# mihaibujanca/dynamicfusion

Measured on AMD Instinct MI355X. Metric: frames/sec integrate+raycast, 640x480->512^3 TSDF, higher is better.
Workload: dtype f32 (fp16 TSDF / u16 weight storage, f64 exp + normalise as in the reference)

## Files before the change

dynamicfusion_amd/csrc/dfusion_internal.h:

```cpp
#pragma once
#include <hip/hip_runtime.h>
#include <stdint.h>
#include <string.h>
#include <memory>
#include <utility>
#include "dfusion.h"
#include "dfusion_device.h"
#include "dfusion_nanoflann.h"

#define DF_BRICK 8
#define DF_WARP_PREFETCH_MARGIN_M 0.05f
#define DF_WARP_PREFETCH_CAP 1024u

#define DF_HIP(expr) do { hipError_t e__ = (expr); if (e__ != hipSuccess) return (int)e__; } while (0)
#define DF_LAUNCH_CHECK() do { hipError_t e__ = hipGetLastError(); if (e__ != hipSuccess) return (int)e__; } while (0)

static inline DfSlab df_slab_or_full(const DfVolume& v, const DfSlab* s)
{
    if (s) return *s;
    DfSlab f; f.z_store0 = 0; f.z_store_n = v.dims[2]; f.z_own0 = 0; f.z_own_n = v.dims[2]; return f;
}
static inline bool df_slab_valid(const DfVolume& v, const DfSlab& s)
{
    return s.z_store_n > 0 && s.z_own_n >= 0 && s.z_store0 >= 0 && s.z_store0 + s.z_store_n <= v.dims[2] &&
// ... 71 lines not shown
    unsigned long long plan_reader[2] = {};
    DfDevBuf<unsigned long long> plan_mask2[2]; DfDevBuf<unsigned int> plan_list2[2]; int pphase = 0; unsigned hphase = 0;
    DfDevBuf<unsigned long long> plan_code2[2];
    DfDevBuf<uint16_t> pyr_mem;
    DfDevBuf<char> solver_ws;
    DfDevBuf<int> graph_nbr; DfDevBuf<float> graph_alpha; DfDevBuf<unsigned int> graph_in_off, graph_in_edge; DfDevBuf<char> graph_ws;
    int graph_kg = 0;
    DfDevBuf<int> pt_ids;
    int pt_image_cols = 0;
    DfDevBuf<DfNfNode> nf_nodes; DfDevBuf<uint16_t> nf_vpos; bool nf_ok = false; int nf_depth = 0;
    DfDevBuf<unsigned int> plan_hist; size_t plan_cap = 0;
    DfDevBuf<uint8_t> blk_state; DfDevBuf<float> blk_wmax; DfDevBuf<uint8_t> blk_alive; DfDevBuf<uint32_t> blk_work, blk_cnt; size_t blk_cap = 0; int blk_phase = 0;
    DfDevBuf<uint8_t> blk_tie;
    DfDevBuf<uint16_t> bm_idx; DfDevBuf<uint32_t> bm_lam, bm_w; DfDevBuf<uint8_t> bm_cnt; size_t bm_cap = 0;
    DfDevBuf<uint32_t> code_tab; size_t code_cap = 0; DfDevBuf<uint32_t> bm_ids; DfDevBuf<uint8_t> bm_coded;
    DfDevBuf<uint32_t> bm_sub_lam, bm_sub_w; DfDevBuf<uint16_t> bm_sub_cnt; DfDevBuf<uint8_t> bm_sub_ok, blk_sub, blk_alive_prev; DfDevBuf<uint32_t> sub_list;
    bool tab_complete = false;
    int tab_sweeps = 0;
    unsigned long long* dbg_swept = nullptr;
    bool alive_valid = false;
    hipStream_t side = nullptr; hipEvent_t ev_fork = nullptr, ev_join = nullptr; bool side_pending = false;
    volatile uint32_t* host_report = nullptr;
    DfDevBuf<char> ext_ws;
    DfDevBuf<char> grow_ws;
};

#define DF_DISPATCH_K(k, ...)                             \
    switch (k) {                                          \
        case 1: { constexpr int K = 1; __VA_ARGS__; } break; \
        case 2: { constexpr int K = 2; __VA_ARGS__; } break; \
        case 3: { constexpr int K = 3; __VA_ARGS__; } break; \
// ... 69 lines not shown
```

dynamicfusion_amd/csrc/dfusion_warp.hip:

```cpp
#include "dfusion_internal.h"
#include "dfusion_pyramid.h"
#include "dfusion_warp_sweep.h"
#include "dfusion_warp_blocks.h"
#include "dfusion_warp_pipe.h"
#include <algorithm>
#include <atomic>
#include <stdlib.h>
#include <stdio.h>
#include <math.h>

__global__ __launch_bounds__(256) void df_dists_max_kernel(const uint16_t* __restrict__ dists, size_t pitch, int cols, int rows,
                                                           float* __restrict__ out)
{
    float m = 0.f;
    for (int i = blockIdx.x * 256 + threadIdx.x; i < cols * rows; i += gridDim.x * 256) {
        const int y = i / cols, x = i - y * cols;
        const float d = h2f_bits(*(const uint16_t*)((const char*)dists + (size_t)y * pitch + 2 * (size_t)x));
        if (!(d <= 3.0e38f)) m = 3.0e38f;
        else m = fmaxf(m, d);
    }
#pragma unroll
    for (int o = 32; o >= 1; o >>= 1) m = fmaxf(m, __shfl_xor(m, o, 64));
    if ((threadIdx.x & 63) == 0) atomicMax((unsigned int*)out, __float_as_uint(m));
}
// ... 132 lines not shown
    wf->blk_phase ^= 1;
    int rc = df_build_listed(wf, cnt, st);
    if (rc) return rc;
    wf->tab_complete = true;
    return DF_OK;
}

static int df_block_verdicts(DfWarpField* wf, DfWarpedArgs& a, int k, unsigned flags, hipStream_t st)
{
    const int nbx = a.tab_ntx * (DF_TAB_TX / 8), nby = a.tab_nty * (DF_TAB_TY / 8), nbz = wf->tab_zn / 8;
    const size_t nblk = (size_t)nbx * nby * nbz;
    if (nblk == 0 || nblk > wf->blk_cap) return DF_E_INVALID;
    const bool use_models = !(flags & DF_WARP_NO_BLOCK_MODEL) && (k == 8 || k == 4);
    const int want_models = !use_models ? 0 : (flags & DF_WARP_BLOCK_MODEL_NOW) ? 2 : wf->tab_sweeps >= 1 ? 1 : 0;
    if (want_models && nblk > wf->bm_cap) {
        wf->bm_cap = 0;
        { int rc = wf->bm_idx.reserve(nblk * DF_BM_NU); if (rc) return rc; }
        { int rc = wf->bm_lam.reserve(nblk * DF_BM_NU); if (rc) return rc; }
        { int rc = wf->bm_w.reserve(nblk * DF_BM_NU); if (rc) return rc; }
        { int rc = wf->bm_cnt.reserve(nblk); if (rc) return rc; }
        wf->bm_cap = nblk;
    }
    if (want_models && k == 8 && (nblk * 512 > wf->code_cap || !wf->bm_ids || !wf->code_tab || !wf->bm_coded || !wf->bm_sub_lam || !wf->bm_sub_w ||
                                  !wf->bm_sub_cnt || !wf->bm_sub_ok || !wf->blk_sub || !wf->sub_list)) {
        wf->code_cap = 0;
        { int rc = wf->bm_ids.reserve(nblk * 64); if (rc) return rc; }
        { int rc = wf->code_tab.reserve(nblk * 512); if (rc) return rc; }
        { int rc = wf->bm_coded.reserve(nblk); if (rc) return rc; }
        DF_HIP(hipMemsetAsync(wf->bm_coded, 0, nblk, st));
        { int rc = wf->bm_sub_lam.reserve(nblk * 8 * DF_BM_NU); if (rc) return rc; }
        { int rc = wf->bm_sub_w.reserve(nblk * 8 * DF_BM_NU); if (rc) return rc; }
        { int rc = wf->bm_sub_cnt.reserve(nblk * 8); if (rc) return rc; }
        { int rc = wf->bm_sub_ok.reserve(nblk); if (rc) return rc; }
        { int rc = wf->blk_sub.reserve(nblk); if (rc) return rc; }
        { int rc = wf->sub_list.reserve(nblk); if (rc) return rc; }
        DF_HIP(hipMemsetAsync(wf->bm_sub_ok, 0, nblk, st));
        wf->code_cap = nblk * 512;
    }
    bool ahead = !(flags & (DF_WARP_NO_PREFETCH | DF_WARP_BLOCK_MODEL_NOW));
    if (ahead) { int rc = df_side_init(wf); if (rc) return rc; }
    if (ahead && !(flags & DF_WARP_STEADY_PREFETCH) && wf->tab_sweeps >= 8 && (wf->tab_sweeps & 7) != 0 && wf->host_report &&
        wf->host_report[0] == 0u && wf->host_report[1] == 0u && wf->host_report[2] == 0u) ahead = false;
    const bool quiet = !ahead && !(flags & (DF_WARP_NO_PREFETCH | DF_WARP_BLOCK_MODEL_NOW));
    const int want_models_policy = want_models;
    const int want_models_now = quiet ? 0 : want_models_policy;
    a.pf_margin = ahead && !wf->tab_complete && wf->tab_sweeps >= 1 ? DF_WARP_PREFETCH_MARGIN_M : 0.f;
    a.pf_cap = DF_WARP_PREFETCH_CAP;
    uint32_t* cnt = wf->blk_cnt + 8 * wf->blk_phase;
    uint32_t* cnt_next = wf->blk_cnt + 8 * (wf->blk_phase ^ 1);
    uint32_t* list_urgent = wf->blk_work, *list_ahead = wf->blk_work + wf->blk_cap, *list_model = wf->blk_work + 2 * wf->blk_cap;
    std::swap(wf->blk_alive, wf->blk_alive_prev);
    const bool codes_exist = k == 8 && wf->bm_cnt && wf->code_tab && wf->bm_ids && wf->bm_coded && wf->code_cap >= nblk * 512;
    const bool sub_verdicts = use_models && wf->bm_cap >= nblk && codes_exist && !(flags & DF_WARP_NO_SUB_VERDICT) && wf->bm_sub_lam && wf->bm_sub_w &&
                              wf->bm_sub_cnt && wf->bm_sub_ok && wf->blk_sub && wf->sub_list && wf->blk_alive_prev;
    if (sub_verdicts) { a.bm_ids = wf->bm_ids; a.bm_sub_lam = wf->bm_sub_lam; a.bm_sub_w = wf->bm_sub_w; a.bm_sub_cnt = wf->bm_sub_cnt; a.bm_sub_ok = wf->bm_sub_ok; }
    hipLaunchKernelGGL(df_block_verdict_kernel, dim3((unsigned)((nblk + 255) / 256)), dim3(256), 0, st, a, wf->rot, wf->node_t, nbx, nby, nbz,
                       wf->blk_state, wf->blk_wmax, wf->brick_thr + wf->off_cap, wf->bx, wf->by, a.tile_wmax != nullptr ? 1 : 0,
                       (use_models && wf->bm_cap >= nblk ? 1 : 0) | (codes_exist ? 2 : 0) | (sub_verdicts ? 4 : 0),
                       want_models_now,
                       wf->tab_complete ? 0 : 1, wf->bm_idx, wf->bm_lam, wf->bm_w, wf->bm_cnt, wf->bm_coded, wf->blk_alive, list_urgent, list_ahead, list_model,
                       cnt, cnt_next, sub_verdicts ? (uint8_t*)wf->blk_sub : nullptr, wf->sub_list, wf->blk_alive_prev);
    a.blk_cnt = cnt; a.host_report = (uint32_t*)wf->host_report; a.sweep_no = (uint32_t)wf->tab_sweeps;
    DF_LAUNCH_CHECK();
#ifdef DF_TRACE_VERDICT
    if (getenv("DF_TRACE_VERDICT_FILE")) {
        DF_HIP(hipStreamSynchronize(st));
        static unsigned long long h[8192 * 4];
        DF_HIP(hipMemcpyFromSymbol(h, HIP_SYMBOL(g_df_vtrace), sizeof(h)));
        FILE* f = fopen(getenv("DF_TRACE_VERDICT_FILE"), "wb");
        if (f) { fwrite(h, 8, 8192 * 4, f); fclose(f); }
    }
#endif
    wf->blk_phase ^= 1;
    auto launch_models = [&](hipStream_t s2) -> int {
        const DfWarpedArgs b = df_table_args(wf);
        static unsigned g8 = 0, g4 = 0;
// ... 6 lines not shown
                                wf->bm_idx, wf->bm_lam, wf->bm_w, wf->bm_cnt, wf->blk_state);
        DF_LAUNCH_CHECK();
        return DF_OK;
    };
    const bool side_work = ahead && (!wf->tab_complete || want_models_now);
    if (side_work) {
        DF_HIP(hipEventRecord(wf->ev_fork, st));
        DF_HIP(hipStreamWaitEvent(wf->side, wf->ev_fork, 0));
        int rc_side = DF_OK;
        if (!wf->tab_complete) rc_side = df_build_listed(wf, cnt, wf->side, 1);
        if (rc_side == DF_OK && want_models_now) rc_side = launch_models(wf->side);
        if (hipEventRecord(wf->ev_join, wf->side) == hipSuccess) wf->side_pending = true;
        else { (void)hipGetLastError(); df_side_drain(wf); if (rc_side == DF_OK) rc_side = (int)hipErrorUnknown; }
        if (rc_side != DF_OK) return rc_side;
    }
    if (sub_verdicts) {
        const unsigned sub_grid = (unsigned)std::min<size_t>((nblk * 8 + 255) / 256, 1024);
        hipLaunchKernelGGL(df_sub_verdict_kernel, dim3(sub_grid), dim3(256), 0, st, a, wf->rot, wf->node_t, nbx, nby, nbz, wf->sub_list, cnt + 5, wf->blk_sub);
        DF_LAUNCH_CHECK();
        a.blk_sub = wf->blk_sub;
    }
    if (!wf->tab_complete) { int rc = df_build_listed(wf, cnt, st, 0); if (rc) return rc; }
    if (want_models_now && !ahead) { int rc = launch_models(st); if (rc) return rc; }
    a.blk_alive = wf->blk_alive; a.bm_nbx = nbx; a.bm_nby = nby;
    wf->alive_valid = true;
    return DF_OK;
}

typedef void (*df_lds_kernel_t)(const DfWarpedArgs, const DfWarpView, int);
struct DfPrepared { DfWarpedArgs a; DfWarpView W; df_lds_kernel_t kern; dim3 grid; unsigned threads; size_t lds; int tiles_x; DfVolume v; DfSlab s; unsigned long long seq; };
DfWarpField::DfWarpField() = default;
DfWarpField::~DfWarpField() = default;
enum { DF_MODE_WHOLE = 0, DF_MODE_PREPARE = 1 };

static int df_integrate_warped_impl(const uint16_t* dists, size_t pitch, int cols, int rows, DfVolume v, const DfSlab* slab,
                                    const float vol2world[12], const float world2cam[12], const float proj[4],
// ... 53 lines not shown
                                    const float vol2world[12], const float world2cam[12], const float proj[4],
                                    DfWarpField* wf, int k, unsigned flags, unsigned long long* n_updated, dfStream stream, int mode)
{
    if (!dists || !vol2world || !world2cam || !proj || !wf || cols <= 0 || rows <= 0 || !df_pitch_ok(pitch, cols, 2) || !df_volume_valid(v)) return DF_E_INVALID;
    if (k < 1 || k > 8 || wf->M < k) return DF_E_INVALID;
    DfSlab s = df_slab_or_full(v, slab);
    if (!df_slab_valid(v, s)) return DF_E_INVALID;
    if (!wf->index_valid || wf->k_built < k || memcmp(wf->geom_dims, v.dims, sizeof(wf->geom_dims)) ||
        memcmp(wf->geom_vs, v.voxel_size, sizeof(wf->geom_vs)) || memcmp(wf->geom_aff, vol2world, sizeof(wf->geom_aff)))
        return DF_E_NO_INDEX;
    if (s.z_own_n == 0) return DF_OK;
    hipStream_t st = (hipStream_t)stream;
    if (mode == DF_MODE_WHOLE) { int rc = df_wait_split_sweep(wf, st); if (rc) return rc; }
    { int rc = df_side_join(wf, st); if (rc) return rc; }
    wf->prep_valid = false;

    DfWarpedArgs a;
    memset(&a, 0, sizeof(a));
    a.vol = (uint32_t*)v.data; a.X = v.dims[0]; a.Y = v.dims[1]; a.Z = v.dims[2];
    a.z_store0 = s.z_store0; a.z_own0 = s.z_own0; a.z_own_n = s.z_own_n;
    a.vsx = v.voxel_size[0]; a.vsy = v.voxel_size[1]; a.vsz = v.voxel_size[2];
    a.vol2world = df_aff(vol2world); a.world2cam = df_aff(world2cam);
    {
        static const float I9[9] = {1.f, 0.f, 0.f, 0.f, 1.f, 0.f, 0.f, 0.f, 1.f};
        a.v2w_identity = memcmp(vol2world, I9, sizeof(I9)) == 0;
    }
    a.P.dists = dists; a.P.pitch = pitch; a.P.cols = cols; a.P.rows = rows;
    a.P.fx = proj[0]; a.P.fy = proj[1]; a.P.cx = proj[2]; a.P.cy = proj[3];
    a.P.trunc = v.trunc_dist; a.P.trunc_inv = 1.f / v.trunc_dist; a.P.max_weight = v.max_weight;
    a.sat_ok = df_sat_trunc_ok(v.trunc_dist) ? 1 : 0;
// ... 199 lines not shown
    if (weights) {
        { int rc = wf->tile_wmax.reserve(ntile); if (rc) return rc; }
        DF_HIP(hipMemsetAsync(wf->tile_wmax, 0, ntile * sizeof(float), st));
    }
    const size_t nblk = (size_t)ntx * (DF_TAB_TX / 8) * nty * (DF_TAB_TY / 8) * (tzn / 8);
    if (nblk > wf->blk_cap) {
        wf->blk_cap = 0;
        { int rc = wf->blk_state.reserve(nblk); if (rc) return rc; }
        { int rc = wf->blk_tie.reserve(nblk); if (rc) return rc; }
        { int rc = wf->blk_wmax.reserve(nblk); if (rc) return rc; }
        { int rc = wf->blk_alive.reserve(nblk); if (rc) return rc; }
        { int rc = wf->blk_alive_prev.reserve(nblk); if (rc) return rc; }
        { int rc = wf->blk_work.reserve(3 * nblk); if (rc) return rc; }
        wf->blk_cap = nblk;
    }
    { int rc = wf->blk_cnt.reserve(16); if (rc) return rc; }
    DF_HIP(hipMemsetAsync(wf->blk_cnt, 0, 16 * sizeof(uint32_t), st));
    DF_HIP(hipMemsetAsync(wf->blk_state, on_demand ? 0 : 1, nblk, st));
    DF_HIP(hipMemsetAsync(wf->blk_tie, 0, nblk, st));
    DF_HIP(hipMemsetAsync(wf->blk_wmax, 0, nblk * sizeof(float), st));
    DF_HIP(hipMemsetAsync(wf->blk_alive, 1, nblk, st));
    DF_HIP(hipMemsetAsync(wf->blk_alive_prev, 1, nblk, st));
    wf->blk_phase = 0;
    wf->tab_z0 = tz0; wf->tab_zn = tzn; wf->tab_k = k; wf->tab_valid = true; wf->w_tab_valid = weights;
    wf->tab_complete = !on_demand; wf->tab_sweeps = 0; wf->alive_valid = false;
    if (on_demand) return DF_OK;
    const DfWarpedArgs a = df_table_args(wf);
    DfWarpView W = df_view(wf);
    dim3 grid((unsigned)(W.bx * W.by), (unsigned)(bz_hi - bz_lo + 1));
    DF_DISPATCH_K(k, df_warp_brick_kernel<K, true><<<grid, dim3(256), 0, st>>>(a, W));
    hipError_t e = hipGetLastError();
    if (e == hipSuccess) e = hipStreamSynchronize(st);
// ... 7 lines not shown
```

dynamicfusion_amd/csrc/dfusion_warp_blocks.h:

```cpp
#pragma once
#include "dfusion_warp_sweep.h"

#define DF_BM_NU 16
#define DF_BM_NONE 0xffu

struct DfIv { float lo, hi; };
__device__ __forceinline__ DfIv iv(float lo, float hi) { DfIv r; r.lo = lo; r.hi = hi; return r; }
__device__ __forceinline__ DfIv iv_add(DfIv a, DfIv b) { return iv(a.lo + b.lo, a.hi + b.hi); }
__device__ __forceinline__ DfIv iv_sub(DfIv a, DfIv b) { return iv(a.lo - b.hi, a.hi - b.lo); }
__device__ __forceinline__ DfIv iv_mul(DfIv a, DfIv b)
{
    const float p0 = a.lo * b.lo, p1 = a.lo * b.hi, p2 = a.hi * b.lo, p3 = a.hi * b.hi;
    return iv(fminf(fminf(p0, p1), fminf(p2, p3)), fmaxf(fmaxf(p0, p1), fmaxf(p2, p3)));
}
__device__ __forceinline__ DfIv iv_sq(DfIv a)
{
    const float l2 = a.lo * a.lo, h2 = a.hi * a.hi;
    return iv((a.lo <= 0.f && a.hi >= 0.f) ? 0.f : fminf(l2, h2), fmaxf(l2, h2));
}
struct DfIv3 { DfIv x, y, z; };
__device__ __forceinline__ DfIv3 iv_cross(const DfIv3& a, const DfIv3& b)
{
    DfIv3 r;
    r.x = iv_sub(iv_mul(a.y, b.z), iv_mul(a.z, b.y));
// ... 285 lines not shown
        for (int i = 0; i < 4; ++i) {
            const size_t at = (size_t)min(e0 + (unsigned)i, n - 1u) * nblk + blk;
            id[i] = bm_idx[at]; lp[i] = bm_lam[at]; wp[i] = bm_w[at];
        }
        float4 r4[4], t4[4];
#pragma unroll
        for (int i = 0; i < 4; ++i) { r4[i] = rot[id[i]]; t4[i] = node_t[id[i]]; }
#pragma unroll
        for (int i = 0; i < 4; ++i) B.add(e0 + (unsigned)i < n, lp[i], wp[i], r4[i], t4[i]);
    }
    const int bx = (int)(blk % (size_t)nbx), by = (int)((blk / (size_t)nbx) % (size_t)nby), bz = (int)(blk / ((size_t)nbx * nby));
    const int x0 = bx * 8, y0 = by * 8, z0 = a.tab_z0 + bz * 8;
    return df_box_dead_finish(a, B, x0, min(x0 + 7, a.X - 1), y0, min(y0 + 7, a.Y - 1), z0, min(z0 + 7, a.Z - 1));
}

__global__ __launch_bounds__(256) void df_sub_verdict_kernel(const DfWarpedArgs a, const float4* __restrict__ rot, const float4* __restrict__ node_t,
                                                             int nbx, int nby, int nbz, const uint32_t* __restrict__ list, const uint32_t* __restrict__ count,
                                                             uint8_t* __restrict__ blk_sub)
{
    const size_t nblk = (size_t)nbx * nby * nbz;
    const unsigned n_lanes = min(*count, (uint32_t)nblk) * 8u;
    for (unsigned base = blockIdx.x * 256u + (threadIdx.x & ~63u); base < n_lanes; base += gridDim.x * 256u) {
    const unsigned i = base + (threadIdx.x & 63u);
    const bool in = i < n_lanes;
    size_t blk = in ? (size_t)list[i >> 3] : 0;
    if (blk >= nblk) blk = 0;
    const unsigned sub = i & 7u, h = sub >> 2, q = sub & 3u;
    const unsigned cr = a.bm_sub_cnt[blk * 8 + sub];
    const uint4* idp = (const uint4*)(a.bm_ids + blk * 64 + q * 16);
    const uint4 i0 = idp[0], i1 = idp[1], i2 = idp[2], i3 = idp[3];
    const unsigned idw[DF_BM_NU] = {i0.x, i0.y, i0.z, i0.w, i1.x, i1.y, i1.z, i1.w, i2.x, i2.y, i2.z, i2.w, i3.x, i3.y, i3.z, i3.w};
    uint32_t lp[DF_BM_NU], wp[DF_BM_NU];
    const size_t at0 = blk * (8 * DF_BM_NU) + sub;
#pragma unroll
    for (int e = 0; e < DF_BM_NU; ++e) { lp[e] = a.bm_sub_lam[at0 + 8 * e]; wp[e] = a.bm_sub_w[at0 + 8 * e]; }
    const unsigned n = in ? min(cr & 0xffu, (unsigned)DF_BM_NU) : 0u, e_ref = min(cr >> 8, (unsigned)DF_BM_NU - 1u);
    unsigned id[DF_BM_NU], id_ref = 0u;
#pragma unroll
    for (int e = 0; e < DF_BM_NU; ++e) {
        id[e] = (unsigned)e < n ? (idw[e] >> (16u * h)) & 0xffffu : 0u;
        id_ref = (unsigned)e == e_ref ? id[e] : id_ref;
    }
    bool live = n != 0u;
    const bool judge = in && n != 0u && a.cull[1] <= 1.0f;
    DfBoxSums B;
    B.ref(rot[id_ref]);
#pragma unroll
    for (int g = 0; g < DF_BM_NU; g += 8) {
        if (g != 0 && __builtin_amdgcn_ballot_w64(judge && n > (unsigned)g) == 0ull) break;
        float4 r4[8], t4[8];
#pragma unroll
        for (int j = 0; j < 8; ++j) { r4[j] = rot[id[g + j]]; t4[j] = node_t[id[g + j]]; }
#pragma unroll
        for (int j = 0; j < 8; ++j) if ((unsigned)(g + j) < n) B.add(true, lp[g + j], wp[g + j], r4[j], t4[j]);
    }
    if (judge) {
        const int bx = (int)(blk % (size_t)nbx), by = (int)((blk / (size_t)nbx) % (size_t)nby), bz = (int)(blk / ((size_t)nbx * nby));
        const int x0 = bx * 8 + (int)(q & 1u) * 4, y0 = by * 8 + (int)(q >> 1) * 4, z0 = a.tab_z0 + bz * 8 + (int)h * 4;
        if (x0 < a.X && y0 < a.Y && z0 < a.Z)
            live = !df_box_dead_finish(a, B, x0, min(x0 + 3, a.X - 1), y0, min(y0 + 3, a.Y - 1), z0, min(z0 + 3, a.Z - 1));
        else live = false;
    }
    const unsigned long long m = __builtin_amdgcn_ballot_w64(live);
    if (in && sub == 0u) blk_sub[blk] = (uint8_t)((unsigned)(m >> ((threadIdx.x & 63u) & ~7u)) & 0xffu);
    }
}

#ifdef DF_TRACE_VERDICT
__device__ unsigned long long g_df_vtrace[8192 * 4];
#define DF_VT(i) do { if ((threadIdx.x & 63) == 0 && blockIdx.x * 4 + (threadIdx.x >> 6) < 8192) g_df_vtrace[(blockIdx.x * 4 + (threadIdx.x >> 6)) * 4 + (i)] = wall_clock64(); } while (0)
#else
#define DF_VT(i) do { } while (0)
#endif
__global__ __launch_bounds__(256) void df_block_verdict_kernel(const DfWarpedArgs a, const float4* __restrict__ rot, const float4* __restrict__ node_t,
                                                               int nbx, int nby, int nbz, uint8_t* __restrict__ blk_state,
                                                               const float* __restrict__ blk_wmax, const float* __restrict__ brick_d1, int vbx, int vby, int zero_skip, int use_models, int want_models,
                                                               int build_on_demand, const uint16_t* __restrict__ bm_idx,
                                                               const uint32_t* __restrict__ bm_lam, const uint32_t* __restrict__ bm_w,
                                                               const uint8_t* __restrict__ bm_cnt, const uint8_t* __restrict__ bm_coded, uint8_t* __restrict__ alive,
                                                               uint32_t* __restrict__ build_list, uint32_t* __restrict__ ahead_list, uint32_t* __restrict__ model_list,
                                                               uint32_t* __restrict__ cnt, uint32_t* __restrict__ cnt_next,
                                                               uint8_t* __restrict__ blk_sub, uint32_t* __restrict__ sub_list, const uint8_t* __restrict__ alive_prev)
{
    __shared__ unsigned s_sub_n, s_sub_base;
    if (threadIdx.x == 0) s_sub_n = 0u;
    const size_t nblk = (size_t)nbx * nby * nbz;
    const size_t blk = (size_t)blockIdx.x * 256 + threadIdx.x;
    DF_VT(0);
    if (blockIdx.x == 0 && threadIdx.x < 8) cnt_next[threadIdx.x] = 0u;
    bool keep = false, near = false, need_build = false, need_ahead = false, need_model = false, need_sub = false;
    int bx = 0, by = 0, bz = 0;
    if (blk < nblk) {
        bx = (int)(blk % (size_t)nbx); by = (int)((blk / (size_t)nbx) % (size_t)nby); bz = (int)(blk / ((size_t)nbx * nby));
        const int x0 = bx * 8, y0 = by * 8, z0 = a.tab_z0 + bz * 8;
        const int own1 = min(a.z_own0 + a.z_own_n, a.Z);
        keep = x0 < a.X && y0 < a.Y && max(z0, a.z_own0) < min(z0 + 8, own1);
        const unsigned st = keep ? blk_state[blk] : 0u;
        if (keep) {
            float wk = a.kf;
            if (zero_skip && st >= 1u) {
                const float wmax = blk_wmax[blk];
                keep = !(wmax * a.cull[3] < DF_ZERO_WEIGHT);
                wk = fminf(wk, wmax * 1.0001f);
            } else if (zero_skip && a.cull[4] < 1.0e30f && a.cull[4] > 0.f) {
// ... 6 lines not shown
            if (keep) {
                const f3 c = aff_mul(a.vol2world, mk3(((float)x0 + 3.5f) * a.vsx, ((float)y0 + 3.5f) * a.vsy, ((float)z0 + 3.5f) * a.vsz));
                if (a.pf_margin > 0.f && st < 2u) {
                    near = !df_tile_culled(a, c, wk, a.pf_margin);
                    keep = near && !df_tile_culled(a, c, wk);
                } else keep = !df_tile_culled(a, c, wk);
            }
        }
        DF_VT(1);
        if (keep && st == 2u && (use_models & 1)) {
            const unsigned n = bm_cnt[blk];
            if (n != DF_BM_NONE && a.cull[1] <= 1.0f) keep = !df_block_box_dead(a, rot, node_t, nbx, nby, nblk, blk, n, bm_idx, bm_lam, bm_w);
        }
        DF_VT(2);
        alive[blk] = keep ? (uint8_t)(1u | ((st == 2u && (use_models & 2) && bm_coded[blk] != 0) ? 2u : 0u)) : (uint8_t)0;
        if (blk_sub) {
            blk_sub[blk] = 0xffu;
            if (keep && st == 2u && (use_models & 4) && a.bm_sub_ok[blk] != 0) {
                const size_t sy = (size_t)nbx, sz = (size_t)nbx * nby;
                const unsigned n0 = bx > 0 ? alive_prev[blk - 1] : 1u, n1 = bx + 1 < nbx ? alive_prev[blk + 1] : 1u, n2 = by > 0 ? alive_prev[blk - sy] : 1u,
                               n3 = by + 1 < nby ? alive_prev[blk + sy] : 1u, n4 = bz > 0 ? alive_prev[blk - sz] : 1u, n5 = bz + 1 < nbz ? alive_prev[blk + sz] : 1u;
                need_sub = n0 == 0u || n1 == 0u || n2 == 0u || n3 == 0u || n4 == 0u || n5 == 0u;
            }
        }
        need_build = keep && build_on_demand && st == 0u;
        need_ahead = !keep && near && build_on_demand && st == 0u;
        need_model = (keep || near) && want_models && (st == 1u || (need_build && want_models > 1));
        if (need_build) blk_state[blk] = 1;
    }
    const unsigned long long mb = __builtin_amdgcn_ballot_w64(need_build), ma = __builtin_amdgcn_ballot_w64(need_ahead), mm = __builtin_amdgcn_ballot_w64(need_model);
    const unsigned long long below = ((unsigned long long)1 << (threadIdx.x & 63)) - 1ull;
    const unsigned code = (unsigned)bx | ((unsigned)by << 10) | ((unsigned)(a.tab_z0 / 8 + bz) << 20);
// ... 4 lines not shown
        if (need_build) build_list[base + (unsigned)__popcll(mb & below)] = code;
    }
    if (ma) {
        unsigned base = 0;
        if ((threadIdx.x & 63) == 0) base = atomicAdd(&cnt[3], (unsigned)__popcll(ma));
        base = (unsigned)__builtin_amdgcn_readfirstlane((int)base);
        const unsigned slot = base + (unsigned)__popcll(ma & below);
        if (need_ahead && slot < a.pf_cap) { ahead_list[slot] = code; blk_state[blk] = 1; }
    }
    if (mm) {
        unsigned base = 0;
        if ((threadIdx.x & 63) == 0) base = atomicAdd(&cnt[1], (unsigned)__popcll(mm));
        base = (unsigned)__builtin_amdgcn_readfirstlane((int)base);
        if (need_model) model_list[base + (unsigned)__popcll(mm & below)] = (unsigned)blk;
    }
    if (blk_sub) {
        const unsigned long long ms = __builtin_amdgcn_ballot_w64(need_sub);
        unsigned wbase = 0;
        __syncthreads();
        if (ms && (threadIdx.x & 63) == 0) wbase = atomicAdd(&s_sub_n, (unsigned)__popcll(ms));
        wbase = (unsigned)__builtin_amdgcn_readfirstlane((int)wbase);
        __syncthreads();
        if (threadIdx.x == 0 && s_sub_n) s_sub_base = atomicAdd(&cnt[5], s_sub_n);
        __syncthreads();
        if (need_sub) sub_list[s_sub_base + wbase + (unsigned)__popcll(ms & below)] = (unsigned)blk;
    }
    DF_VT(3);
}

__global__ __launch_bounds__(256) void df_blocks_unbuilt_kernel(int nbx, int nby, int nbz, int vbx, int vby, int tab_bz0, uint8_t* __restrict__ blk_state,
                                                                uint32_t* __restrict__ build_list, uint32_t* __restrict__ cnt,
                                                                uint32_t* __restrict__ cnt_next)
{
    const size_t nblk = (size_t)nbx * nby * nbz;
    const size_t blk = (size_t)blockIdx.x * 256 + threadIdx.x;
    if (blockIdx.x == 0 && threadIdx.x < 8) cnt_next[threadIdx.x] = 0u;
    bool need = false;
    int bx = 0, by = 0, bz = 0;
    if (blk < nblk) {
        bx = (int)(blk % (size_t)nbx); by = (int)((blk / (size_t)nbx) % (size_t)nby); bz = (int)(blk / ((size_t)nbx * nby));
        need = blk_state[blk] == 0 && bx < vbx && by < vby;
        if (blk_state[blk] == 0) blk_state[blk] = 1;
// ... 11 lines not shown
```

dynamicfusion_amd/csrc/dfusion_warp_index.hip:

```cpp
#include "dfusion_internal.h"
#include "dfusion_warp_sweep.h"
#include <math.h>

struct DfIndexGeom {
    int X, Y, Z; int bx, by, bz;
    float vsx, vsy, vsz;
    DfAff vol2world;
    float r2x;
};

#define DF_SUPER 4
#define DF_SUPER_CAP 1024
template <int K>
__device__ __forceinline__ float df_wave_kth_pop(float (&bd)[K], float* first)
{
    const int lane = threadIdx.x & 63;
    float dk2 = 0.f;
#pragma unroll
    for (int r = 0; r < K; ++r) {
        const float m = wave_min_f32(bd[0]);
        dk2 = m;
        if (r == 0) *first = m;
        const unsigned long long who = __ballot(bd[0] == m);
        const int first = __ffsll((long long)who) - 1;
// ... 238 lines not shown
        for (int i = 0; i < 3; ++i)
            wf->geom_inv[9 + i] = (float)-((d[3 * i] * m[9] + d[3 * i + 1] * m[10] + d[3 * i + 2] * m[11]) / det);
    }
    return DF_OK;
}

extern "C" int dfusion_warp_build_index(DfWarpField* wf, DfVolume v, const DfSlab* slab, const float vol2world[12], int k,
                                        unsigned flags, dfStream stream)
{
    if (!wf || !vol2world || wf->M <= 0 || k < 1 || k > 8 || wf->M < k) return DF_E_INVALID;
    if (v.dims[0] <= 0 || v.dims[1] <= 0 || v.dims[2] <= 0) return DF_E_INVALID;
    DfSlab sl = df_slab_or_full(v, slab);
    if (sl.z_own_n < 0 || sl.z_own0 < 0 || sl.z_own0 + sl.z_own_n > v.dims[2]) return DF_E_INVALID;
    hipStream_t st = (hipStream_t)stream;
    df_side_drain(wf);
    wf->prep_valid = false;
    { int rc = df_index_bricks(wf, v, vol2world, k, st); if (rc) return rc; }
    wf->index_flags = flags; wf->index_slab = sl;
    wf->index_valid = true;
    wf->tab_valid = false;
    wf->w_tab_valid = false;
    if (flags & (DF_INDEX_VOXEL_TABLE | DF_INDEX_WEIGHT_TABLE))
        return df_build_voxel_table(wf, v, sl, vol2world, k, (flags & DF_INDEX_WEIGHT_TABLE) != 0,
                                    (flags & DF_INDEX_TABLES_ON_DEMAND) != 0 && (flags & DF_INDEX_WEIGHT_TABLE) != 0, st);
    return DF_OK;
}

extern "C" int dfusion_warp_index_info(const DfWarpField* wf, unsigned long long* total_entries, unsigned int* n_bricks, int* k_built)
{
    if (!wf || !wf->index_valid) return DF_E_NO_INDEX;
// ... 55 lines not shown
    }
    wf->index_valid = false;
    DfVolume v; memset(&v, 0, sizeof(v));
    memcpy(v.dims, wf->geom_dims, sizeof(v.dims)); memcpy(v.voxel_size, wf->geom_vs, sizeof(v.voxel_size));
    float aff[12]; memcpy(aff, wf->geom_aff, sizeof(aff));
    { int rc = df_index_bricks(wf, v, aff, wf->k_built, st); if (rc) return rc; }
    wf->index_valid = true;
    if (!tabs) return DF_OK;
    const DfWarpedArgs a = df_table_args(wf);
    const int nbz = wf->tab_zn / 8;
    const size_t nblk = (size_t)a.bm_nbx * a.bm_nby * nbz;
    hipLaunchKernelGGL(df_grow_dirty_kernel, dim3((unsigned)((nblk + 255) / 256)), dim3(256), 0, st, old_off, old_list, wf->brick_off, wf->brick_list,
                       wf->bx, wf->by, wf->bz, a.bm_nbx, a.bm_nby, nbz, wf->tab_z0 / DF_BRICK, wf->blk_state, a.blk_wmax, wf->blk_tie);
    DF_LAUNCH_CHECK();
    wf->alive_valid = false; wf->tab_complete = false;
    if (!((wf->index_flags & DF_INDEX_TABLES_ON_DEMAND) && wf->w_tab_valid)) {
        int rc = df_tables_complete(wf, st);
        if (rc) return rc;
    }
    DF_HIP(hipStreamSynchronize(st));
    return DF_OK;
}
```

dynamicfusion_amd/csrc/dfusion_warp_nodes.hip:

```cpp
#include "dfusion_internal.h"
#include <utility>
#include <vector>

__global__ __launch_bounds__(256) void df_pack_nodes_kernel(const float* __restrict__ pos, const float* __restrict__ dq,
                                                            const float* __restrict__ sigma, int M,
                                                            float4* __restrict__ pos_sigma, float4* __restrict__ rot,
                                                            float4* __restrict__ dual, float4* __restrict__ node_t, float4* __restrict__ rt)
{
    int j = blockIdx.x * 256 + threadIdx.x;
    if (j >= M) return;
    if (pos) pos_sigma[j] = make_float4(pos[3 * j], pos[3 * j + 1], pos[3 * j + 2], sigma[j]);
    quat r, d;
    r.w = dq[8 * j]; r.x = dq[8 * j + 1]; r.y = dq[8 * j + 2]; r.z = dq[8 * j + 3];
    d.w = dq[8 * j + 4]; d.x = dq[8 * j + 5]; d.y = dq[8 * j + 6]; d.z = dq[8 * j + 7];
    quat t = dq_get_translation(r, d);
    rot[j] = make_float4(r.w, r.x, r.y, r.z);
    dual[j] = make_float4(d.w, d.x, d.y, d.z);
    node_t[j] = make_float4(t.w, t.x, t.y, t.z);
    rt[2 * j] = rot[j]; rt[2 * j + 1] = node_t[j];
}

__global__ __launch_bounds__(256) void df_node_bounds_kernel(const float4* __restrict__ rot, const float4* __restrict__ node_t,
                                                             int M, float* __restrict__ bounds)
{
// ... 217 lines not shown
    return DF_OK;
}

extern "C" int dfusion_warp_set_nodes(DfWarpField* wf, const float* pos, const float* dq, const float* sigma, int M,
                                      dfStream stream)
{
    if (!wf || !pos || !dq || !sigma || M <= 0 || M > 65535) return DF_E_INVALID;
    df_side_drain(wf);
    wf->prep_valid = false;
    int rc = df_warp_reserve(wf, M);
    if (rc) return rc;
    wf->M = M;
    wf->graph_kg = 0;
    wf->index_valid = false;
    wf->tab_valid = false; wf->w_tab_valid = false;
    rc = df_warp_pack(wf, pos, dq, sigma, (hipStream_t)stream);
    if (rc) return rc;
    return df_warp_build_tie_tree(wf, (hipStream_t)stream);
}

extern "C" int dfusion_warp_set_transforms(DfWarpField* wf, const float* dq, dfStream stream)
{
    if (!wf || !dq || wf->M <= 0) return DF_E_INVALID;
    return df_warp_pack(wf, nullptr, dq, nullptr, (hipStream_t)stream);
}

DfWarpView df_view(const DfWarpField* wf)
{
    DfWarpView W;
    W.pos_sigma = wf->pos_sigma; W.rot = wf->rot; W.dual = wf->dual; W.node_t = wf->node_t; W.rt = wf->rt; W.M = wf->M;
// ... 5 lines not shown
```

Measured before the change: 2013.

## Fuse sub-verdict into block-verdict launch using previous call's sub list

Removes the separate sub-verdict kernel launch. The block-verdict kernel now gets extra workgroups that judge sub-blocks using the list built in the previous call. That list is kept in double-buffered sub lists and blk_sub arrays, with rotating counters, and an invalidation key forces a fallback whenever geometry, nodes or call order change. The sub-verdict loop is also rewritten to prefetch node ids, lambdas and weights in groups of four, and it adds a blk_state check. The cost is that verdicts lag one call behind the list, so blocks that newly qualify stay conservatively fully live (0xff) for that call, and state management gets more complex.

```diff
diff --git a/dynamicfusion_amd/csrc/dfusion_internal.h b/dynamicfusion_amd/csrc/dfusion_internal.h
--- a/dynamicfusion_amd/csrc/dfusion_internal.h
+++ b/dynamicfusion_amd/csrc/dfusion_internal.h
@@ -109,7 +109,8 @@
     DfDevBuf<uint8_t> blk_tie;
     DfDevBuf<uint16_t> bm_idx; DfDevBuf<uint32_t> bm_lam, bm_w; DfDevBuf<uint8_t> bm_cnt; size_t bm_cap = 0;
     DfDevBuf<uint32_t> code_tab; size_t code_cap = 0; DfDevBuf<uint32_t> bm_ids; DfDevBuf<uint8_t> bm_coded;
-    DfDevBuf<uint32_t> bm_sub_lam, bm_sub_w; DfDevBuf<uint16_t> bm_sub_cnt; DfDevBuf<uint8_t> bm_sub_ok, blk_sub, blk_alive_prev; DfDevBuf<uint32_t> sub_list;
+    DfDevBuf<uint32_t> bm_sub_lam, bm_sub_w; DfDevBuf<uint16_t> bm_sub_cnt; DfDevBuf<uint8_t> bm_sub_ok, blk_sub2[2], blk_alive_prev; DfDevBuf<uint32_t> sub_list2[2];
+    unsigned judge_no = 0; bool sub_void = true; int judge_key[6] = {}; unsigned long long call_no = 0, judge_call = 0;
     bool tab_complete = false;
     int tab_sweeps = 0;
     unsigned long long* dbg_swept = nullptr;
diff --git a/dynamicfusion_amd/csrc/dfusion_warp.hip b/dynamicfusion_amd/csrc/dfusion_warp.hip
--- a/dynamicfusion_amd/csrc/dfusion_warp.hip
+++ b/dynamicfusion_amd/csrc/dfusion_warp.hip
@@ -170,7 +170,7 @@
     const bool use_models = !(flags & DF_WARP_NO_BLOCK_MODEL) && (k == 8 || k == 4);
     const int want_models = !use_models ? 0 : (flags & DF_WARP_BLOCK_MODEL_NOW) ? 2 : wf->tab_sweeps >= 1 ? 1 : 0;
     if (want_models && nblk > wf->bm_cap) {
-        wf->bm_cap = 0;
+        wf->bm_cap = 0; wf->sub_void = true;
         { int rc = wf->bm_idx.reserve(nblk * DF_BM_NU); if (rc) return rc; }
         { int rc = wf->bm_lam.reserve(nblk * DF_BM_NU); if (rc) return rc; }
         { int rc = wf->bm_w.reserve(nblk * DF_BM_NU); if (rc) return rc; }
@@ -178,7 +178,7 @@
         wf->bm_cap = nblk;
     }
     if (want_models && k == 8 && (nblk * 512 > wf->code_cap || !wf->bm_ids || !wf->code_tab || !wf->bm_coded || !wf->bm_sub_lam || !wf->bm_sub_w ||
-                                  !wf->bm_sub_cnt || !wf->bm_sub_ok || !wf->blk_sub || !wf->sub_list)) {
+                                  !wf->bm_sub_cnt || !wf->bm_sub_ok || !wf->blk_sub2[0] || !wf->blk_sub2[1] || !wf->sub_list2[0] || !wf->sub_list2[1])) {
         wf->code_cap = 0;
         { int rc = wf->bm_ids.reserve(nblk * 64); if (rc) return rc; }
         { int rc = wf->code_tab.reserve(nblk * 512); if (rc) return rc; }
@@ -188,8 +188,12 @@
         { int rc = wf->bm_sub_w.reserve(nblk * 8 * DF_BM_NU); if (rc) return rc; }
         { int rc = wf->bm_sub_cnt.reserve(nblk * 8); if (rc) return rc; }
         { int rc = wf->bm_sub_ok.reserve(nblk); if (rc) return rc; }
-        { int rc = wf->blk_sub.reserve(nblk); if (rc) return rc; }
-        { int rc = wf->sub_list.reserve(nblk); if (rc) return rc; }
+        wf->sub_void = true;
+        for (int i = 0; i < 2; ++i) {
+            { int rc = wf->blk_sub2[i].reserve(nblk); if (rc) return rc; }
+            { int rc = wf->sub_list2[i].reserve(nblk); if (rc) return rc; }
+            DF_HIP(hipMemsetAsync(wf->blk_sub2[i], 0xff, wf->blk_sub2[i].cap, st));
+        }
         DF_HIP(hipMemsetAsync(wf->bm_sub_ok, 0, nblk, st));
         wf->code_cap = nblk * 512;
     }
@@ -208,14 +212,36 @@
     std::swap(wf->blk_alive, wf->blk_alive_prev);
     const bool codes_exist = k == 8 && wf->bm_cnt && wf->code_tab && wf->bm_ids && wf->bm_coded && wf->code_cap >= nblk * 512;
     const bool sub_verdicts = use_models && wf->bm_cap >= nblk && codes_exist && !(flags & DF_WARP_NO_SUB_VERDICT) && wf->bm_sub_lam && wf->bm_sub_w &&
-                              wf->bm_sub_cnt && wf->bm_sub_ok && wf->blk_sub && wf->sub_list && wf->blk_alive_prev;
+                              wf->bm_sub_cnt && wf->bm_sub_ok && wf->blk_sub2[0] && wf->blk_sub2[1] && wf->sub_list2[0] && wf->sub_list2[1] && wf->blk_alive_prev &&
+                              wf->blk_cnt.cap >= 19;
     if (sub_verdicts) { a.bm_ids = wf->bm_ids; a.bm_sub_lam = wf->bm_sub_lam; a.bm_sub_w = wf->bm_sub_w; a.bm_sub_cnt = wf->bm_sub_cnt; a.bm_sub_ok = wf->bm_sub_ok; }
-    hipLaunchKernelGGL(df_block_verdict_kernel, dim3((unsigned)((nblk + 255) / 256)), dim3(256), 0, st, a, wf->rot, wf->node_t, nbx, nby, nbz,
-                       wf->blk_state, wf->blk_wmax, wf->brick_thr + wf->off_cap, wf->bx, wf->by, a.tile_wmax != nullptr ? 1 : 0,
-                       (use_models && wf->bm_cap >= nblk ? 1 : 0) | (codes_exist ? 2 : 0) | (sub_verdicts ? 4 : 0),
-                       want_models_now,
-                       wf->tab_complete ? 0 : 1, wf->bm_idx, wf->bm_lam, wf->bm_w, wf->bm_cnt, wf->bm_coded, wf->blk_alive, list_urgent, list_ahead, list_model,
-                       cnt, cnt_next, sub_verdicts ? (uint8_t*)wf->blk_sub : nullptr, wf->sub_list, wf->blk_alive_prev);
+    const unsigned nV = (unsigned)((nblk + 255) / 256);
+    unsigned nS = 0, jn = wf->judge_no;
+    bool list_void = true;
+    if (sub_verdicts) {
+        const int key[6] = {wf->tab_z0, nbx, nby, nbz, a.z_own0, a.z_own_n};
+        list_void = wf->sub_void || wf->judge_call + 1 != wf->call_no || memcmp(key, wf->judge_key, sizeof(key)) != 0;
+        memcpy(wf->judge_key, key, sizeof(key)); wf->judge_call = wf->call_no;
+        if (!list_void) nS = (unsigned)std::min<size_t>((nblk * 8 + 255) / 256, 1024);
+        wf->sub_void = false; ++wf->judge_no;
+    }
+    uint32_t* sub_cnt = wf->blk_cnt + 16;
+    DfJudgeArgs j;
+    memset(&j, 0, sizeof(j));
+    j.rot = wf->rot; j.node_t = wf->node_t; j.nbx = nbx; j.nby = nby; j.nbz = nbz; j.blk_state = wf->blk_state; j.blk_wmax = wf->blk_wmax;
+    j.brick_d1 = wf->brick_thr + wf->off_cap; j.vbx = wf->bx; j.vby = wf->by; j.zero_skip = a.tile_wmax != nullptr ? 1 : 0;
+    j.use_models = (use_models && wf->bm_cap >= nblk ? 1 : 0) | (codes_exist ? 2 : 0) | (sub_verdicts ? 4 : 0);
+    j.want_models = want_models_now; j.build_on_demand = wf->tab_complete ? 0 : 1;
+    j.bm_idx = wf->bm_idx; j.bm_lam = wf->bm_lam; j.bm_w = wf->bm_w; j.bm_cnt = wf->bm_cnt; j.bm_coded = wf->bm_coded; j.alive = wf->blk_alive;
+    j.build_list = list_urgent; j.ahead_list = list_ahead; j.model_list = list_model; j.cnt = cnt; j.cnt_next = cnt_next;
+    j.alive_prev = wf->blk_alive_prev; j.nV = nV; j.list_void = list_void ? 1 : 0;
+    if (sub_verdicts) {
+        j.blk_sub_next = wf->blk_sub2[(jn + 1) & 1]; j.blk_sub_cur = wf->blk_sub2[jn & 1];
+        j.sub_list = wf->sub_list2[jn & 1]; j.sub_cnt_fill = sub_cnt + jn % 3; j.sub_cnt_zero = sub_cnt + (jn + 1) % 3;
+        j.sub_prev = wf->sub_list2[(jn + 1) & 1]; j.sub_cnt_prev = sub_cnt + (jn + 2) % 3;
+    }
+    hipLaunchKernelGGL(df_block_verdict_kernel, dim3(nV + nS), dim3(256), 0, st, a, j);
+    if (sub_verdicts) a.blk_sub = wf->blk_sub2[jn & 1];
     a.blk_cnt = cnt; a.host_report = (uint32_t*)wf->host_report; a.sweep_no = (uint32_t)wf->tab_sweeps;
     DF_LAUNCH_CHECK();
 #ifdef DF_TRACE_VERDICT
@@ -252,12 +278,6 @@
         else { (void)hipGetLastError(); df_side_drain(wf); if (rc_side == DF_OK) rc_side = (int)hipErrorUnknown; }
         if (rc_side != DF_OK) return rc_side;
     }
-    if (sub_verdicts) {
-        const unsigned sub_grid = (unsigned)std::min<size_t>((nblk * 8 + 255) / 256, 1024);
-        hipLaunchKernelGGL(df_sub_verdict_kernel, dim3(sub_grid), dim3(256), 0, st, a, wf->rot, wf->node_t, nbx, nby, nbz, wf->sub_list, cnt + 5, wf->blk_sub);
-        DF_LAUNCH_CHECK();
-        a.blk_sub = wf->blk_sub;
-    }
     if (!wf->tab_complete) { int rc = df_build_listed(wf, cnt, st, 0); if (rc) return rc; }
     if (want_models_now && !ahead) { int rc = launch_models(st); if (rc) return rc; }
     a.blk_alive = wf->blk_alive; a.bm_nbx = nbx; a.bm_nby = nby;
@@ -341,6 +361,7 @@
     if (mode == DF_MODE_WHOLE) { int rc = df_wait_split_sweep(wf, st); if (rc) return rc; }
     { int rc = df_side_join(wf, st); if (rc) return rc; }
     wf->prep_valid = false;
+    ++wf->call_no;
 
     DfWarpedArgs a;
     memset(&a, 0, sizeof(a));
@@ -570,8 +591,9 @@
         { int rc = wf->blk_work.reserve(3 * nblk); if (rc) return rc; }
         wf->blk_cap = nblk;
     }
-    { int rc = wf->blk_cnt.reserve(16); if (rc) return rc; }
-    DF_HIP(hipMemsetAsync(wf->blk_cnt, 0, 16 * sizeof(uint32_t), st));
+    { int rc = wf->blk_cnt.reserve(20); if (rc) return rc; }
+    DF_HIP(hipMemsetAsync(wf->blk_cnt, 0, 20 * sizeof(uint32_t), st));
+    wf->sub_void = true;
     DF_HIP(hipMemsetAsync(wf->blk_state, on_demand ? 0 : 1, nblk, st));
     DF_HIP(hipMemsetAsync(wf->blk_tie, 0, nblk, st));
     DF_HIP(hipMemsetAsync(wf->blk_wmax, 0, nblk * sizeof(float), st));
diff --git a/dynamicfusion_amd/csrc/dfusion_warp_blocks.h b/dynamicfusion_amd/csrc/dfusion_warp_blocks.h
--- a/dynamicfusion_amd/csrc/dfusion_warp_blocks.h
+++ b/dynamicfusion_amd/csrc/dfusion_warp_blocks.h
@@ -323,45 +323,54 @@
     return df_box_dead_finish(a, B, x0, min(x0 + 7, a.X - 1), y0, min(y0 + 7, a.Y - 1), z0, min(z0 + 7, a.Z - 1));
 }
 
-__global__ __launch_bounds__(256) void df_sub_verdict_kernel(const DfWarpedArgs a, const float4* __restrict__ rot, const float4* __restrict__ node_t,
-                                                             int nbx, int nby, int nbz, const uint32_t* __restrict__ list, const uint32_t* __restrict__ count,
-                                                             uint8_t* __restrict__ blk_sub)
+template <int G>
+__device__ __forceinline__ void df_sub_verdict_role(const DfWarpedArgs& a, const float4* __restrict__ rot, const float4* __restrict__ node_t,
+                                                    int nbx, int nby, int nbz, const uint32_t* __restrict__ list, const uint32_t* __restrict__ count,
+                                                    const uint8_t* __restrict__ blk_state, uint8_t* __restrict__ blk_sub, unsigned wg, unsigned n_wg)
 {
     const size_t nblk = (size_t)nbx * nby * nbz;
     const unsigned n_lanes = min(*count, (uint32_t)nblk) * 8u;
-    for (unsigned base = blockIdx.x * 256u + (threadIdx.x & ~63u); base < n_lanes; base += gridDim.x * 256u) {
+    const unsigned wave = (unsigned)__builtin_amdgcn_readfirstlane((int)(threadIdx.x >> 6));
+    for (unsigned base = (wg * 4u + wave) * 64u; base < n_lanes; base += n_wg * 256u) {
     const unsigned i = base + (threadIdx.x & 63u);
     const bool in = i < n_lanes;
     size_t blk = in ? (size_t)list[i >> 3] : 0;
     if (blk >= nblk) blk = 0;
     const unsigned sub = i & 7u, h = sub >> 2, q = sub & 3u;
-    const unsigned cr = a.bm_sub_cnt[blk * 8 + sub];
-    const uint4* idp = (const uint4*)(a.bm_ids + blk * 64 + q * 16);
-    const uint4 i0 = idp[0], i1 = idp[1], i2 = idp[2], i3 = idp[3];
-    const unsigned idw[DF_BM_NU] = {i0.x, i0.y, i0.z, i0.w, i1.x, i1.y, i1.z, i1.w, i2.x, i2.y, i2.z, i2.w, i3.x, i3.y, i3.z, i3.w};
-    uint32_t lp[DF_BM_NU], wp[DF_BM_NU];
+    const uint32_t* idp = a.bm_ids + blk * 64 + q * 16;
     const size_t at0 = blk * (8 * DF_BM_NU) + sub;
-#pragma unroll
-    for (int e = 0; e < DF_BM_NU; ++e) { lp[e] = a.bm_sub_lam[at0 + 8 * e]; wp[e] = a.bm_sub_w[at0 + 8 * e]; }
-    const unsigned n = in ? min(cr & 0xffu, (unsigned)DF_BM_NU) : 0u, e_ref = min(cr >> 8, (unsigned)DF_BM_NU - 1u);
-    unsigned id[DF_BM_NU], id_ref = 0u;
-#pragma unroll
-    for (int e = 0; e < DF_BM_NU; ++e) {
-        id[e] = (unsigned)e < n ? (idw[e] >> (16u * h)) & 0xffffu : 0u;
-        id_ref = (unsigned)e == e_ref ? id[e] : id_ref;
-    }
+    unsigned idn[G]; uint32_t lpn[G], wpn[G];
+#pragma unroll
+    for (int j = 0; j < G; ++j) { idn[j] = idp[j]; lpn[j] = a.bm_sub_lam[at0 + 8 * j]; wpn[j] = a.bm_sub_w[at0 + 8 * j]; }
+    const unsigned cr_all = a.bm_sub_cnt[blk * 8 + sub];
+    const bool has = in && blk_state[blk] == 2 && a.bm_sub_ok[blk] != 0;
+    const unsigned cr = has ? cr_all : 0u;
+    const unsigned n = min(cr & 0xffu, (unsigned)DF_BM_NU), e_ref = min(cr >> 8, (unsigned)DF_BM_NU - 1u);
     bool live = n != 0u;
-    const bool judge = in && n != 0u && a.cull[1] <= 1.0f;
+    const bool judge = has && n != 0u && a.cull[1] <= 1.0f;
     DfBoxSums B;
-    B.ref(rot[id_ref]);
-#pragma unroll
-    for (int g = 0; g < DF_BM_NU; g += 8) {
-        if (g != 0 && __builtin_amdgcn_ballot_w64(judge && n > (unsigned)g) == 0ull) break;
-        float4 r4[8], t4[8];
-#pragma unroll
-        for (int j = 0; j < 8; ++j) { r4[j] = rot[id[g + j]]; t4[j] = node_t[id[g + j]]; }
-#pragma unroll
-        for (int j = 0; j < 8; ++j) if ((unsigned)(g + j) < n) B.add(true, lp[g + j], wp[g + j], r4[j], t4[j]);
+    B.ref(rot[judge && e_ref < n ? (idp[e_ref] >> (16u * h)) & 0xffffu : 0u]);
+#pragma unroll
+    for (unsigned g = 0; g < (unsigned)DF_BM_NU; g += (unsigned)G) {
+        if (__builtin_amdgcn_ballot_w64(judge && n > g) == 0ull) break;
+        unsigned id[G]; uint32_t lp[G], wp[G];
+#pragma unroll
+        for (int j = 0; j < G; ++j) { id[j] = idn[j]; lp[j] = lpn[j]; wp[j] = wpn[j]; }
+        if (g + (unsigned)G < (unsigned)DF_BM_NU) {
+#pragma unroll
+            for (int j = 0; j < G; ++j) {
+                const unsigned e = g + (unsigned)G + (unsigned)j;
+                idn[j] = idp[e]; lpn[j] = a.bm_sub_lam[at0 + 8 * e]; wpn[j] = a.bm_sub_w[at0 + 8 * e];
+            }
+        }
+        float4 r4[G], t4[G];
+#pragma unroll
+        for (int j = 0; j < G; ++j) {
+            id[j] = judge && g + (unsigned)j < n ? (id[j] >> (16u * h)) & 0xffffu : 0u;
+            r4[j] = rot[id[j]]; t4[j] = node_t[id[j]];
+        }
+#pragma unroll
+        for (int j = 0; j < G; ++j) if (g + (unsigned)j < n) B.add(true, lp[j], wp[j], r4[j], t4[j]);
     }
     if (judge) {
         const int bx = (int)(blk % (size_t)nbx), by = (int)((blk / (size_t)nbx) % (size_t)nby), bz = (int)(blk / ((size_t)nbx * nby));
@@ -371,7 +380,7 @@
         else live = false;
     }
     const unsigned long long m = __builtin_amdgcn_ballot_w64(live);
-    if (in && sub == 0u) blk_sub[blk] = (uint8_t)((unsigned)(m >> ((threadIdx.x & 63u) & ~7u)) & 0xffu);
+    if (has && sub == 0u) blk_sub[blk] = (uint8_t)((unsigned)(m >> ((threadIdx.x & 63u) & ~7u)) & 0xffu);
     }
 }
 
@@ -381,7 +390,7 @@
 #else
 #define DF_VT(i) do { } while (0)
 #endif
-__global__ __launch_bounds__(256) void df_block_verdict_kernel(const DfWarpedArgs a, const float4* __restrict__ rot, const float4* __restrict__ node_t,
+__device__ __forceinline__ void df_block_verdict_role(const DfWarpedArgs& a, const float4* __restrict__ rot, const float4* __restrict__ node_t,
                                                                int nbx, int nby, int nbz, uint8_t* __restrict__ blk_state,
                                                                const float* __restrict__ blk_wmax, const float* __restrict__ brick_d1, int vbx, int vby, int zero_skip, int use_models, int want_models,
                                                                int build_on_demand, const uint16_t* __restrict__ bm_idx,
@@ -389,7 +398,9 @@
                                                                const uint8_t* __restrict__ bm_cnt, const uint8_t* __restrict__ bm_coded, uint8_t* __restrict__ alive,
                                                                uint32_t* __restrict__ build_list, uint32_t* __restrict__ ahead_list, uint32_t* __restrict__ model_list,
                                                                uint32_t* __restrict__ cnt, uint32_t* __restrict__ cnt_next,
-                                                               uint8_t* __restrict__ blk_sub, uint32_t* __restrict__ sub_list, const uint8_t* __restrict__ alive_prev)
+                                                               uint8_t* __restrict__ blk_sub_next, uint8_t* __restrict__ blk_sub_cur, int list_void,
+                                                               uint32_t* __restrict__ sub_list, uint32_t* __restrict__ sub_cnt_fill,
+                                                               uint32_t* __restrict__ sub_cnt_zero, const uint8_t* __restrict__ alive_prev)
 {
     __shared__ unsigned s_sub_n, s_sub_base;
     if (threadIdx.x == 0) s_sub_n = 0u;
@@ -397,6 +408,7 @@
     const size_t blk = (size_t)blockIdx.x * 256 + threadIdx.x;
     DF_VT(0);
     if (blockIdx.x == 0 && threadIdx.x < 8) cnt_next[threadIdx.x] = 0u;
+    if (blockIdx.x == 0 && threadIdx.x == 8 && blk_sub_next) *sub_cnt_zero = 0u;
     bool keep = false, near = false, need_build = false, need_ahead = false, need_model = false, need_sub = false;
     int bx = 0, by = 0, bz = 0;
     if (blk < nblk) {
@@ -433,8 +445,9 @@
         }
         DF_VT(2);
         alive[blk] = keep ? (uint8_t)(1u | ((st == 2u && (use_models & 2) && bm_coded[blk] != 0) ? 2u : 0u)) : (uint8_t)0;
-        if (blk_sub) {
-            blk_sub[blk] = 0xffu;
+        if (blk_sub_next) {
+            blk_sub_next[blk] = 0xffu;
+            if (list_void) blk_sub_cur[blk] = 0xffu;
             if (keep && st == 2u && (use_models & 4) && a.bm_sub_ok[blk] != 0) {
                 const size_t sy = (size_t)nbx, sz = (size_t)nbx * nby;
                 const unsigned n0 = bx > 0 ? alive_prev[blk - 1] : 1u, n1 = bx + 1 < nbx ? alive_prev[blk + 1] : 1u, n2 = by > 0 ? alive_prev[blk - sy] : 1u,
@@ -469,18 +482,41 @@
         base = (unsigned)__builtin_amdgcn_readfirstlane((int)base);
         if (need_model) model_list[base + (unsigned)__popcll(mm & below)] = (unsigned)blk;
     }
-    if (blk_sub) {
+    if (blk_sub_next) {
         const unsigned long long ms = __builtin_amdgcn_ballot_w64(need_sub);
         unsigned wbase = 0;
         __syncthreads();
         if (ms && (threadIdx.x & 63) == 0) wbase = atomicAdd(&s_sub_n, (unsigned)__popcll(ms));
         wbase = (unsigned)__builtin_amdgcn_readfirstlane((int)wbase);
         __syncthreads();
-        if (threadIdx.x == 0 && s_sub_n) s_sub_base = atomicAdd(&cnt[5], s_sub_n);
+        if (threadIdx.x == 0 && s_sub_n) s_sub_base = atomicAdd(sub_cnt_fill, s_sub_n);
         __syncthreads();
         if (need_sub) sub_list[s_sub_base + wbase + (unsigned)__popcll(ms & below)] = (unsigned)blk;
     }
     DF_VT(3);
+}
+
+#define DF_SUB_ROLE_G 4
+struct DfJudgeArgs {
+    const float4* rot; const float4* node_t; int nbx, nby, nbz; uint8_t* blk_state; const float* blk_wmax; const float* brick_d1;
+    int vbx, vby, zero_skip, use_models, want_models, build_on_demand;
+    const uint16_t* bm_idx; const uint32_t* bm_lam; const uint32_t* bm_w; const uint8_t* bm_cnt; const uint8_t* bm_coded; uint8_t* alive;
+    uint32_t* build_list; uint32_t* ahead_list; uint32_t* model_list; uint32_t* cnt; uint32_t* cnt_next;
+    uint8_t* blk_sub_next; uint8_t* blk_sub_cur; int list_void; uint32_t* sub_list; uint32_t* sub_cnt_fill; uint32_t* sub_cnt_zero;
+    const uint8_t* alive_prev;
+    unsigned nV; const uint32_t* sub_prev; const uint32_t* sub_cnt_prev;
+};
+__global__ __launch_bounds__(256, 4) void df_block_verdict_kernel(const DfWarpedArgs a, const DfJudgeArgs j)
+{
+    if (blockIdx.x >= j.nV) {
+        df_sub_verdict_role<DF_SUB_ROLE_G>(a, j.rot, j.node_t, j.nbx, j.nby, j.nbz, j.sub_prev, j.sub_cnt_prev, j.blk_state, j.blk_sub_cur,
+                                           blockIdx.x - j.nV, gridDim.x - j.nV);
+        return;
+    }
+    df_block_verdict_role(a, j.rot, j.node_t, j.nbx, j.nby, j.nbz, j.blk_state, j.blk_wmax, j.brick_d1, j.vbx, j.vby, j.zero_skip, j.use_models,
+                          j.want_models, j.build_on_demand, j.bm_idx, j.bm_lam, j.bm_w, j.bm_cnt, j.bm_coded, j.alive, j.build_list, j.ahead_list,
+                          j.model_list, j.cnt, j.cnt_next, j.blk_sub_next, j.blk_sub_cur, j.list_void, j.sub_list, j.sub_cnt_fill, j.sub_cnt_zero,
+                          j.alive_prev);
 }
 
 __global__ __launch_bounds__(256) void df_blocks_unbuilt_kernel(int nbx, int nby, int nbz, int vbx, int vby, int tab_bz0, uint8_t* __restrict__ blk_state,
diff --git a/dynamicfusion_amd/csrc/dfusion_warp_index.hip b/dynamicfusion_amd/csrc/dfusion_warp_index.hip
--- a/dynamicfusion_amd/csrc/dfusion_warp_index.hip
+++ b/dynamicfusion_amd/csrc/dfusion_warp_index.hip
@@ -276,6 +276,7 @@
     if (sl.z_own_n < 0 || sl.z_own0 < 0 || sl.z_own0 + sl.z_own_n > v.dims[2]) return DF_E_INVALID;
     hipStream_t st = (hipStream_t)stream;
     df_side_drain(wf);
+    wf->sub_void = true;
     wf->prep_valid = false;
     { int rc = df_index_bricks(wf, v, vol2world, k, st); if (rc) return rc; }
     wf->index_flags = flags; wf->index_slab = sl;
@@ -361,6 +362,7 @@
                        wf->bx, wf->by, wf->bz, a.bm_nbx, a.bm_nby, nbz, wf->tab_z0 / DF_BRICK, wf->blk_state, a.blk_wmax, wf->blk_tie);
     DF_LAUNCH_CHECK();
     wf->alive_valid = false; wf->tab_complete = false;
+    wf->sub_void = true;
     if (!((wf->index_flags & DF_INDEX_TABLES_ON_DEMAND) && wf->w_tab_valid)) {
         int rc = df_tables_complete(wf, st);
         if (rc) return rc;
diff --git a/dynamicfusion_amd/csrc/dfusion_warp_nodes.hip b/dynamicfusion_amd/csrc/dfusion_warp_nodes.hip
--- a/dynamicfusion_amd/csrc/dfusion_warp_nodes.hip
+++ b/dynamicfusion_amd/csrc/dfusion_warp_nodes.hip
@@ -255,6 +255,7 @@
     wf->graph_kg = 0;
     wf->index_valid = false;
     wf->tab_valid = false; wf->w_tab_valid = false;
+    wf->sub_void = true;
     rc = df_warp_pack(wf, pos, dq, sigma, (hipStream_t)stream);
     if (rc) return rc;
     return df_warp_build_tie_tree(wf, (hipStream_t)stream);
```

Result: slower. 1973 (-2.0%).
